# entn-at/tf-kaldi-speaker

Hardware: AMD Instinct MI355X
Metric: utterances/sec x-vector extraction (30-dim x 300-frame) (higher is better)
Workload: dtype f16+fp6-cross(f32-split); 1 GPU; tdnn x-vector (tdnn6_dense), statistics_pooling, 256 utt/GPU/step of 300 frames x 30 dims; batch_per_gpu=256, frames=300, node=tdnn6_dense, precision=f16f6, parallelism=utterance-shard x1, launch=stream launches

## Files before the change

### tf-kaldi-speaker_amd/csrc/api_forward.hip

```cpp
#include "xv_model.h"

using namespace xv;
using namespace xv::api;

namespace {

struct Run {
  xv_handle* h;
  const xv_plan* p;
  const float* feats;
  int feat_ld;
  float* out;
  char* ws;
  hipStream_t s;
  int f16;
  int B;
  const int32_t* off;
  char* raw(int64_t o) const { return o >= 0 ? ws + o : nullptr; }
  float* f32(int64_t o) const { return reinterpret_cast<float*>(raw(o)); }
  const float* in(int64_t o) const { return o == -2 ? feats : f32(o); }
  float* dst(const PlanStep& st) const { return st.out_off >= 0 ? f32(st.out_off) : out; }
  int* ovf() const { return static_cast<int*>(h->ovf_flag.p); }
};

// ... 45 lines not shown
    if (st.compact()) {
      a.arow = static_cast<const int32_t*>(r.p->d_rowmaps.p) + r.p->rowmap_off[st.arow];
      a.a_pitch = L.cin;
      a.a_off = L.mode == 1 ? 0 : (Sin + 1) * L.cin;
    }
    a.ntaps = L.mode == 1 ? 3 : 1;
    a.ktap = L.mode == 1 ? 3 * L.cin : (L.mode == 2 ? L.cin : L.Fin * L.cin);
    a.tap_stride = Sin * L.cin;
    a.cin = a.K;
  }
  if (op.in1 > 0) { a.R = r.in(st.in1_off); a.ldr = L.cout; }
  if (st.fuse_att == 1) {
    a.Y = nullptr;
    a.att_part = r.f32(st.out_off);
    a.att_ld = st.att_ld;
    a.att_heads = d.att_num_heads;
    a.att_q = static_cast<const float*>(h->query_eff.p);
  } else if (st.fuse_att == 2) {
    a.Y = nullptr;
    a.pool_part = r.f32(st.out_off);
    a.pool_row2utt = static_cast<const int32_t*>(r.p->d_row2utt.p);
    a.pool_slotbase = static_cast<const int32_t*>(r.p->d_slotbase.p);
    a.pool_w = r.f32(st.att_w_off);
    a.pool_heads = d.att_num_heads;
    a.pool_split = d.att_split_value;
    a.pool_dvh = d.att_split_value ? L.cout / d.att_num_heads : L.cout;
    a.pool_odim = h->pool_dim / 2;
  }
  if (st.fuse_pool) {
    a.Y = nullptr;
    a.pool_part = r.f32(st.out_off);
    a.pool_row2utt = static_cast<const int32_t*>(r.p->d_row2utt.p);
    a.pool_slotbase = static_cast<const int32_t*>(r.p->d_slotbase.p);
  }
  if (st.out_sb_off >= 0) {
    a.Ysb = r.raw(st.out_sb_off);
    a.ldsb = sb_ld(L.cout);
    if (st.out_off < 0 && !st.to_out) a.Y = nullptr;
  }
  return a;
}

int gemm_clear_border(const Run& r, const PlanStep& st, const Layer& L, const Value& vo) {
  xv_handle* h = r.h;
  const size_t head = (size_t)vo.grid_S + 1;
  const size_t rows0 = st.grid_cover && L.mode != 4 ? head : (st.grid_cover ? 0 : (size_t)st.rows_out + vo.grid_S);
  if (st.compact() || st.trows()) {
    XV_HIP(h, launch_grid_zero_border(r.p->dev_offsets(st.lvl_out), r.B, st.frames_out, vo.grid_F, vo.grid_S, L.cout / 4,
                                      sb_ld(L.cout) / 4, r.f32(st.out_off), r.raw(st.out_sb_off), r.s));
  } else if (rows0 > 0) {
    if (st.out_off >= 0) XV_HIP(h, hipMemsetAsync(r.raw(st.out_off), 0, rows0 * L.cout * 4, r.s));
    if (st.out_sb_off >= 0) XV_HIP(h, hipMemsetAsync(r.raw(st.out_sb_off), 0, rows0 * sb_ld(L.cout) * 4, r.s));
  }
  return XV_OK;
}

int launch_conv0(const Run& r, const PlanStep& st, const Layer& L, const Value& vo, GemmArgs& a) {
  xv_handle* h = r.h;
  if (st.scratch_off < 0) return fail(h, XV_ERR_STATE, "conv0 has no scratch");
  a.cin = 32; a.K = 32;
  const bool direct = L.use_split && !st.to_out && st.stage == L.final_stage() && L.cout % 8 == 0 &&
                      (st.out_sb_off < 0 || L.cout % 32 == 0) && L.cout <= 256 && L.wdir.p;
  if (direct) {
    XV_HIP(h, launch_conv0_direct(r.feats, r.feat_ld, r.off, r.B, L.Fout, vo.grid_S, L.cout, st.M, static_cast<const float*>(L.wdir.p),
                                  L.act, L.d_alpha(), r.f32(st.out_off), r.raw(st.out_sb_off), sb_ld(L.cout), r.f16, r.ovf(),
                                  a.sb_mul, r.s));
  } else if (L.use_split) {
    XV_HIP(h, launch_im2col2d_sb(r.feats, r.feat_ld, r.off, r.B, L.Fout, vo.grid_S, st.M, r.raw(st.scratch_off), r.f16, r.ovf(), r.s));
    a.Xsb = r.raw(st.scratch_off); a.ldsbx = 32; a.Wsb = L.wsb.p; a.Wfr = L.wfr.p;
    XV_HIP(h, launch_gemm_bf16x3(a, r.s));
  } else {
    XV_HIP(h, launch_im2col2d_f32(r.feats, r.feat_ld, r.off, r.B, L.Fout, vo.grid_S, st.M, r.f32(st.scratch_off), r.s));
    a.X = r.f32(st.scratch_off); a.ldx = 32;
    XV_HIP(h, launch_gemm_f32(a, true, r.s));
  }
  return XV_OK;
}

int launch_first_layer(const Run& r, const PlanStep& st, const Layer& L, GemmArgs& a) {
  xv_handle* h = r.h;
  if (st.scratch_off < 0) return fail(h, XV_ERR_STATE, "im2col layer has no scratch");
  a.Xsb = r.raw(st.scratch_off);
  a.Wsb = L.wsb.p; a.Wfr = L.wfr.p;
  if (L.cin_pad) {
    XV_HIP(h, launch_im2col_sb(r.feats, r.feat_ld, L.cin, 1, st.rows_in, r.raw(st.scratch_off), L.cin_pad, r.f16, r.ovf(), r.s));
    a.ldsbx = L.cin_pad;
    a.cin = L.cin_pad;
    a.K = L.w * L.cin_pad;
    a.ysb_f6 = st.out_f6 ? 1 : 0;
  } else {
    XV_HIP(h, launch_im2col_sb(r.feats, r.feat_ld, L.cin, L.w, st.M, r.raw(st.scratch_off), L.Kpad, r.f16, r.ovf(), r.s));
    a.ldsbx = L.Kpad;
    a.cin = a.K;
  }
  if (r.f16) XV_HIP(h, launch_feat_utt_guard(r.feats, r.feat_ld, L.cin, r.off, r.B, r.ovf(), r.s));
  XV_HIP(h, launch_gemm_bf16x3(a, r.s));
  return XV_OK;
}

int launch_two_unit(const Run& r, const PlanStep& st, const Op& op, const Layer& L, GemmArgs& a) {
  xv_handle* h = r.h;
  if (st.in0_sb_off < 0 || st.scratch_off < 0) return fail(h, XV_ERR_STATE, "f16f6 layer %s has no input / scratch", L.kernel_name.c_str());
  if (st.in_f6) {
    a.Xsb = r.raw(st.in0_sb_off);
  } else {
    XV_HIP(h, launch_f6_from_sb(r.raw(st.in0_sb_off), r.raw(st.scratch_off), st.rows_in, sb_ld(L.cin) / 32, r.s));
    a.Xsb = r.raw(st.scratch_off);
    XV_HIP(h, hipMemsetAsync(r.raw(st.scratch_off) + st.rows_in * (int64_t)sb_ld(L.cin) * 4, 0, (size_t)8 * sb_ld(L.cin) * 4, r.s));
  }
  a.ysb_f6 = st.out_f6 ? 1 : 0;
  a.ldsbx = sb_ld(L.cin);
  a.Wfr = L.wf6m.p;
  a.Wx6 = L.wf6x.p;
  if (st.trows()) {
    const int64_t Sin = h->values[op.in0].grid_S;
    a.a_pitch = 0; a.a_off = 0; a.arow = nullptr; a.ntaps = 0; a.ktap = 0; a.tap_stride = 0;
    a.ldsbx = Sin * L.cin;
    a.cin = 3 * L.cin;
    a.K = 9 * L.cin;
    a.nbin = L.Fout;
    a.bin_x_bytes = (int64_t)L.cin * 4;
    if (a.Ysb) a.Ysb = static_cast<char*>(a.Ysb) + (int64_t)a.ldsb * 4;
    if (a.Y) a.Y += a.ldy;
    if (a.R) a.R += a.ldr;
  }
  if (st.tail_mt > 0 && st.scratch2_off >= 0) {
    a.tail_mt = st.tail_mt;
    a.ksplit = st.ksplit;
    a.partial = r.f32(st.scratch2_off);
  }
  XV_HIP(h, launch_gemm_f16f6(a, r.s));
  return XV_OK;
}

int launch_split(const Run& r, const PlanStep& st, const Layer& L, GemmArgs& a) {
  xv_handle* h = r.h;
  if (st.in0_sb_off < 0) return fail(h, XV_ERR_STATE, "split layer %s has no split-blocked input", L.kernel_name.c_str());
  a.Xsb = r.raw(st.in0_sb_off);
  a.ldsbx = L.mode == 0 ? sb_ld(L.cin) : 0;
  a.Wsb = L.wsb.p; a.Wfr = L.wfr.p;
  a.ysb_f6 = st.out_f6 ? 1 : 0;
  if (st.tail_mt > 0 && st.scratch_off >= 0) {
    a.tail_mt = st.tail_mt;
    a.ksplit = st.ksplit;
    a.partial = r.f32(st.scratch_off);
  }
  XV_HIP(h, launch_gemm_bf16x3(a, r.s));
  return XV_OK;
}

int launch_fp32(const Run& r, const PlanStep& st, const Op& op, const Layer& L, GemmArgs& a) {
  xv_handle* h = r.h;
  if (st.ksplit > 1 && st.scratch_off >= 0) {
    a.ksplit = st.ksplit;
    a.partial = r.f32(st.scratch_off);
  }
  const bool aligned = op.in0 != 0 && (a.ldx % 4 == 0) && (a.K % 4 == 0);
  if (L.mode != 0 && !aligned)
    return fail(h, XV_ERR_UNSUPPORTED, "resnet convolution %s needs channel counts that are multiples of 4", L.kernel_name.c_str());
  XV_HIP(h, launch_gemm_f32(a, aligned, r.s));
  return XV_OK;
}

int run_gemm(const Run& r, const PlanStep& st, const Op& op) {
  xv_handle* h = r.h;
  const Layer& L = h->layers[op.layer];
  const Value& vo = h->values[op.out];
  GemmArgs a = gemm_args(r, st, op, L);
  int rc = vo.grid_F > 0 ? gemm_clear_border(r, st, L, vo) : XV_OK;
  if (rc != XV_OK) return rc;
  if (L.mode == 4) rc = launch_conv0(r, st, L, vo, a);
  else if (L.im2col) rc = launch_first_layer(r, st, L, a);
  else if (L.use_f6) rc = launch_two_unit(r, st, op, L, a);
  else if (L.use_split) rc = launch_split(r, st, L, a);
  else rc = launch_fp32(r, st, op, L, a);
  if (rc != XV_OK) return rc;
  if (st.unpad_to_out)
    XV_HIP(h, launch_grid_unpad_n(r.f32(st.out_off), r.p->dev_offsets(st.lvl_out), r.B, vo.grid_F, vo.grid_S, vo.cols, st.frames_out,
// ... 208 lines not shown
```

### tf-kaldi-speaker_amd/csrc/api_weights.hip

```cpp
#include "xv_model.h"

using namespace xv;
using namespace xv::api;

namespace {

constexpr double kBnEps = 1e-3;

uint16_t f32_to_bf16_rn(float f) {
  uint32_t u;
  memcpy(&u, &f, 4);
  if ((u & 0x7fffffffu) > 0x7f800000u) return (uint16_t)((u >> 16) | 0x40);
  u += 0x7fffu + ((u >> 16) & 1u);
  return (uint16_t)(u >> 16);
}
float bf16_to_f32(uint16_t b) {
  uint32_t u = (uint32_t)b << 16;
  float f;
  memcpy(&f, &u, 4);
  return f;
}
uint16_t f32_to_f16_rn(float f) {
  const _Float16 h = (_Float16)f;
  uint16_t u;
// ... 244 lines not shown
  return XV_OK;
}

void choose_kernels(xv_handle* h) {
  for (const Op& op : h->ops) {
    if (op.kind != OP_GEMM) continue;
    Layer& L = h->layers[op.layer];
    const Value& vin = h->values[op.in0];
    const bool bf = h->desc.precision != XV_PREC_F32;
    if (L.mode == 0) {
      L.im2col = bf && op.in0 == 0;
      L.cin_pad = (L.im2col && L.w <= 9) ? (int)align_up(L.cin, 32) : 0;
      L.use_split = L.im2col || (bf && vin.frame_level && (L.w == 1 || (L.cin % 32 == 0 && L.w <= 9)));
      L.use_f6 = h->desc.precision == XV_PREC_F16F6 && L.use_split && !L.im2col && (L.w == 5 || L.w == 7 || L.w == 9) &&
                 L.cin % 128 == 0 && L.cout % 4 == 0;
    } else {
      L.use_split = bf && (L.mode == 4 || L.cin % 32 == 0);
      L.use_f6 = h->desc.precision == XV_PREC_F16F6 && h->opt_grid_f6 && L.mode == 1 && L.use_split && L.sw == 1 && L.st == 1 &&
                 L.cin % 128 == 0 && L.cout % 128 == 0;
    }
    if (L.use_f6 && f6_block_spread(h, op, L) > kF6MaxSpread) L.use_f6 = false;
  }
  if (h->desc.precision == XV_PREC_F16X3 || h->desc.precision == XV_PREC_F16F6) {
    for (const Op& op : h->ops) {
      if (op.kind == OP_GEMM) {
        Layer& L = h->layers[op.layer];
        L.in_exp = (L.use_split && !L.im2col && L.mode != 4 && op.in0 > 0) ? h->values[op.in0].sb_exp : 0;
        L.out_exp = act_exponent(h, L);
        h->values[op.out].sb_exp = L.out_exp;
      } else if (op.kind == OP_GRID_MAXPOOL) {
        h->values[op.out].sb_exp = h->values[op.in0].sb_exp;
      }
    }
  }
}

}

extern "C" {

int xv_finalize(xv_handle* h) {
  if (!h) return fail(nullptr, XV_ERR_INVALID, "xv_finalize: null handle");
  std::lock_guard<std::mutex> lk(h->mu);
  if (h->finalized) return XV_OK;
  for (const auto& kv : h->tensors)
    if (!kv.second.set) return fail(h, XV_ERR_MISSING_TENSOR, "variable '%s' was never set", kv.first.c_str());
  choose_kernels(h);
  DeviceGuard g(h->device);
  if (!g.ok) return fail(h, XV_ERR_HIP, "cannot select HIP device %d", h->device);
  for (auto& L : h->layers) {
    const int rc = upload_layer(h, L);
    if (rc != XV_OK) return rc;
  }
  if (h->desc.pooling_type == XV_POOL_SELF_ATTENTION) {
    const auto& q = T(h, std::string(h->desc.network_type == XV_NET_ETDNN ? "etdnn/" : "tdnn/") + "attention/query").data;
    XV_HIP(h, h->query.alloc(q.size() * sizeof(float)));
    XV_HIP(h, hipMemcpy(h->query.p, q.data(), q.size() * sizeof(float), hipMemcpyHostToDevice));
    {
      const int H = h->desc.att_num_heads, dkh = h->att_dk_h;
      h->key_npad = (int)align_up(h->att_dk, 128);
      std::vector<float> qe((size_t)H * h->key_npad, 0.f);
      for (int hd = 0; hd < H; ++hd)
        for (int d = 0; d < dkh; ++d) {
          const int n = h->desc.att_split_key ? hd * dkh + d : d;
          qe[(size_t)hd * h->key_npad + n] = q[(size_t)hd * dkh + d];
        }
      XV_HIP(h, h->query_eff.alloc(qe.size() * sizeof(float)));
      XV_HIP(h, hipMemcpy(h->query_eff.p, qe.data(), qe.size() * sizeof(float), hipMemcpyHostToDevice));
    }
    if (h->desc.att_apply_nonlinear) {
      const int n = h->pool_dim;
      std::vector<double> s, t;
      bn_fold(h, h->post_bn_scope, n, s, t);
      std::vector<float> vec((size_t)3 * n, 0.f);
      for (int i = 0; i < n; ++i) { vec[i] = (float)s[i]; vec[(size_t)n + i] = (float)t[i]; }
      if (!h->post_alpha_name.empty()) {
        const auto& a = T(h, h->post_alpha_name).data;
        for (int i = 0; i < n; ++i) vec[(size_t)2 * n + i] = a[i];
      }
      XV_HIP(h, h->post_vec.alloc(vec.size() * sizeof(float)));
      XV_HIP(h, hipMemcpy(h->post_vec.p, vec.data(), vec.size() * sizeof(float), hipMemcpyHostToDevice));
    }
  }
  XV_HIP(h, h->ovf_flag.alloc((kFlagWords + kFeatMaxSlots) * sizeof(int)));
  XV_HIP(h, hipMemset(h->ovf_flag.p, 0, (kFlagWords + kFeatMaxSlots) * sizeof(int)));
  XV_HIP(h, hipDeviceSynchronize());
  for (auto& kv : h->tensors) { kv.second.data.clear(); kv.second.data.shrink_to_fit(); }
  h->finalized = true;
  return XV_OK;
}

int xv_check_overflow(xv_handle* h, int reset) {
  if (!h) return fail(nullptr, XV_ERR_INVALID, "xv_check_overflow: null handle");
  if (!h->finalized || !h->ovf_flag.p) return 0;
  DeviceGuard g(h->device);
  std::vector<int32_t> w((size_t)kFlagWords + kFeatMaxSlots);
  XV_HIP(h, hipMemcpy(w.data(), h->ovf_flag.p, w.size() * sizeof(int32_t), hipMemcpyDeviceToHost));
  int32_t v[2] = {w[0], w[1]};
  for (int i = 0; i < kFeatMaxSlots; ++i) v[1] = std::max(v[1], w[(size_t)kFlagWords + i]);
  if (w[kUttSmallWord]) v[1] = w[kUttSmallWord];
  if (reset) XV_HIP(h, hipMemset(h->ovf_flag.p, 0, w.size() * sizeof(int32_t)));
  return xv_flags_decode(v);
}

int xv_flags_decode(const int32_t* flags) {
  if (!flags) return XV_ERR_INVALID;
  if (flags[0]) return 1;
  if (flags[1] > 0) {
    float mx;
    memcpy(&mx, &flags[1], 4);
    if (mx < 0.00390625f) return 2;
  }
  return 0;
}

int xv_flags_async(xv_handle* h, int32_t* host_flags, void* stream) {
  if (!h || !host_flags) return fail(h, XV_ERR_INVALID, "xv_flags_async: null argument");
  if (!h->finalized || !h->ovf_flag.p) { host_flags[0] = host_flags[1] = 0; return XV_OK; }
  DeviceGuard g(h->device);
  hipStream_t s = static_cast<hipStream_t>(stream);
  hipPointerAttribute_t attr;
  if (hipPointerGetAttributes(&attr, host_flags) == hipSuccess && attr.type == hipMemoryTypeHost) {
    XV_HIP(h, launch_flags_snapshot(static_cast<int*>(h->ovf_flag.p), host_flags, s));
    return XV_OK;
  }
  (void)hipGetLastError();
  XV_HIP(h, launch_flags_snapshot(static_cast<int*>(h->ovf_flag.p), static_cast<int*>(h->ovf_flag.p) + 2, s));
  XV_HIP(h, hipMemcpyAsync(host_flags, static_cast<int*>(h->ovf_flag.p) + 2, 2 * sizeof(int32_t), hipMemcpyDeviceToHost, s));
  return XV_OK;
}

}
```

### tf-kaldi-speaker_amd/csrc/gemm_f32.hip

```cpp
#include <mutex>

#include "xv_epilogue.h"

namespace xv {

constexpr int BM = 128, BN = 128, BK = 32;
constexpr int LDT = BK + 4;
constexpr int TILE_F = BM * LDT;

template <int FORM>
__global__ __launch_bounds__(256, 2) void gemm_f32_kernel(GemmArgs p, int nMt, int nNt, int kper) {
  extern __shared__ __attribute__((aligned(16))) float smem[];
  float* As = smem;
  float* Bs = smem + 2 * TILE_F;

  const int tid = threadIdx.x;
  const int lane = tid & 63, wave = tid >> 6;
  const int wm = wave >> 1, wn = wave & 1;
  const int r32 = lane & 31, h = lane >> 5;

  const int ntiles = nMt * nNt;
  const int slice = blockIdx.x / ntiles;
  const int tile = xcd_remap(blockIdx.x - slice * ntiles, ntiles);
  const int mt = tile / nNt, nt = tile - mt * nNt;
// ... 32 lines not shown
        }
      } else {
        const int m = m0 + row;
        f32x4 v = {0.f, 0.f, 0.f, 0.f};
        if (m < p.M) {
#pragma unroll
          for (int e = 0; e < 4; ++e) {
            const int kk = k + e;
            if (kk < p.K) {
              const int dr = kk / p.cin;
              v[e] = p.X[(int64_t)(m + dr) * p.ldx + (kk - dr * p.cin)];
            }
          }
        }
        ra[i] = v;
      }
    }
  };
  auto store_tiles = [&](int buf) {
#pragma unroll
    for (int i = 0; i < 4; ++i) {
      const int row = lr + 32 * i;
      *reinterpret_cast<f32x4*>(As + buf * TILE_F + row * LDT + c4 * 4) = ra[i];
      *reinterpret_cast<f32x4*>(Bs + buf * TILE_F + row * LDT + c4 * 4) = rb[i];
    }
  };

  f32x16 acc[2][2];
#pragma unroll
  for (int i = 0; i < 2; ++i)
#pragma unroll
    for (int j = 0; j < 2; ++j)
#pragma unroll
      for (int e = 0; e < 16; ++e) acc[i][j][e] = 0.f;

  load_tiles(kt0);
  store_tiles(0);
  __syncthreads();

  const float* a_base = As + (wm * 64 + r32) * LDT + 4 * h;
  const float* b_base = Bs + (wn * 64 + r32) * LDT + 4 * h;

  for (int kt = kt0; kt < nk; ++kt) {
    const int cur = (kt - kt0) & 1;
    if (kt + 1 < nk) load_tiles(kt + 1);
    const float* ap = a_base + cur * TILE_F;
    const float* bp = b_base + cur * TILE_F;
#pragma unroll
    for (int q = 0; q < BK / 8; ++q) {
      f32x4 a0 = *reinterpret_cast<const f32x4*>(ap + q * 8);
      f32x4 a1 = *reinterpret_cast<const f32x4*>(ap + 32 * LDT + q * 8);
      f32x4 b0 = *reinterpret_cast<const f32x4*>(bp + q * 8);
      f32x4 b1 = *reinterpret_cast<const f32x4*>(bp + 32 * LDT + q * 8);
#pragma unroll
      for (int j = 0; j < 4; ++j) {
        acc[0][0] = __builtin_amdgcn_mfma_f32_32x32x2f32(b0[j], a0[j], acc[0][0], 0, 0, 0);
        acc[0][1] = __builtin_amdgcn_mfma_f32_32x32x2f32(b0[j], a1[j], acc[0][1], 0, 0, 0);
        acc[1][0] = __builtin_amdgcn_mfma_f32_32x32x2f32(b1[j], a0[j], acc[1][0], 0, 0, 0);
        acc[1][1] = __builtin_amdgcn_mfma_f32_32x32x2f32(b1[j], a1[j], acc[1][1], 0, 0, 0);
      }
    }
    if (kt + 1 < nk) store_tiles(cur ^ 1);
    __syncthreads();
  }

  store_wave_tile(p, acc, m0 + wm * 64, n0 + wn * 64, lane, wave, reinterpret_cast<char*>(smem));
}

__global__ void splitk_reduce_kernel(GemmArgs p) {
  const int64_t total = (int64_t)p.M * p.N;
  for (int64_t i = (int64_t)blockIdx.x * blockDim.x + threadIdx.x; i < total; i += (int64_t)gridDim.x * blockDim.x) {
    const int m = (int)(i / p.N), n = (int)(i - (int64_t)m * p.N);
    float acc = 0.f;
    for (int s = 0; s < p.ksplit; ++s) acc += p.partial[((int64_t)s * p.M + m) * p.Npad + n];
    bool zero;
    const int orow = out_row(p, m, zero);
    if (orow < 0) continue;
    float v = fmaf(acc, p.scale[n], p.shift[n]);
    if (p.R) v += p.R[(int64_t)orow * p.ldr + n];
    p.Y[(int64_t)orow * p.ldy + n] = zero ? 0.f : apply_act(v, p.act, p.alpha ? p.alpha[n] : 0.f);
  }
}

int gemm_f32_ksplit(int M, int Kpad, int Npad) {
  if (M > 512) return 1;
  const int tiles = ((M + BM - 1) / BM) * (Npad / BN), nk = Kpad / BK;
  int s = 512 / (tiles > 0 ? tiles : 1);
  if (s > nk / 4) s = nk / 4;
  return s < 2 ? 1 : s;
}

hipError_t launch_gemm_f32(const GemmArgs& a, bool aligned, hipStream_t s) {
  if (a.M <= 0) return hipSuccess;
  const int nMt = (a.M + BM - 1) / BM, nNt = a.Npad / BN;
  const int ks = (a.ksplit > 1 && a.partial && !a.Ysb && !a.pool_part) ? a.ksplit : 1;
  const int nk_all = a.Kpad / BK;
  const int kper = (nk_all + ks - 1) / ks;
  const size_t smem = (size_t)4 * TILE_F * sizeof(float);
  static std::mutex init_mu;
  static bool attr_set[64] = {};
  int dev = 0;
  if (hipGetDevice(&dev) != hipSuccess) dev = 0;
  std::lock_guard<std::mutex> init_lock(init_mu);
  if (!attr_set[dev & 63]) {
    hipError_t e = hipFuncSetAttribute(reinterpret_cast<const void*>(gemm_f32_kernel<2>),
                                       hipFuncAttributeMaxDynamicSharedMemorySize, (int)smem);
    if (e != hipSuccess) return e;
    e = hipFuncSetAttribute(reinterpret_cast<const void*>(gemm_f32_kernel<1>),
                                       hipFuncAttributeMaxDynamicSharedMemorySize, (int)smem);
    if (e != hipSuccess) return e;
    e = hipFuncSetAttribute(reinterpret_cast<const void*>(gemm_f32_kernel<0>),
                            hipFuncAttributeMaxDynamicSharedMemorySize, (int)smem);
    if (e != hipSuccess) return e;
    attr_set[dev & 63] = true;
  }
  GemmArgs b = a;
  b.ksplit = ks;
  dim3 grid(nMt * nNt * ks), block(256);
  if (aligned && a.a_pitch)
    hipLaunchKernelGGL(gemm_f32_kernel<2>, grid, block, smem, s, b, nMt, nNt, kper);
  else if (aligned)
    hipLaunchKernelGGL(gemm_f32_kernel<1>, grid, block, smem, s, b, nMt, nNt, kper);
  else
    hipLaunchKernelGGL(gemm_f32_kernel<0>, grid, block, smem, s, b, nMt, nNt, kper);
  hipError_t e = hipGetLastError();
  if (e != hipSuccess || ks == 1) return e;
  const int64_t total = (int64_t)a.M * a.N;
  const int blocks = (int)((total + 255) / 256 > 1024 ? 1024 : (total + 255) / 256);
  hipLaunchKernelGGL(splitk_reduce_kernel, dim3(blocks), dim3(256), 0, s, b);
  return hipGetLastError();
}

}
```

### tf-kaldi-speaker_amd/csrc/pool.hip

```cpp
#include "xv_epilogue.h"

namespace xv {


__device__ __forceinline__ float act_apply(float v, int act, float alpha) {
  switch (act) {
    case ACT_RELU: return fmaxf(v, 0.0f);
    case ACT_LRELU: return fmaxf(v, kLreluAlpha * v);
    case ACT_PRELU: return fmaxf(v, 0.0f) + alpha * (v - fabsf(v)) * 0.5f;
    case ACT_TANH: return tanhf(v);
    default: return v;
  }
}

__device__ __forceinline__ float wave_sum(float v) {
#pragma unroll
  for (int o = 32; o > 0; o >>= 1) v += __shfl_xor(v, o, 64);
  return v;
}
__device__ __forceinline__ float wave_max(float v) {
#pragma unroll
  for (int o = 32; o > 0; o >>= 1) v = fmaxf(v, __shfl_xor(v, o, 64));
  return v;
}
// ... 307 lines not shown
  const int h = min(split ? oc / dvh : oc / (odim / H), H - 1);
  const int r0 = off0[b] - b * ctx, r1 = off0[b + 1] - (b + 1) * ctx;
  const int t0 = r0 >> 6, t1 = (r1 - 1) >> 6;
  const int64_t base = (int64_t)slotbase[b];
  float mean = 0.f;
  for (int t = t0; t <= t1; ++t) mean += part[((base + t) * 2) * odim + oc];
  float var = 0.f;
  for (int t = t0; t <= t1; ++t) {
    const float w = s0[(base + t) * H + h];
    const float d = w > 0.f ? part[((base + t) * 2) * odim + oc] / w - mean : 0.f;
    var += part[((base + t) * 2 + 1) * odim + oc] + w * d * d;
  }
  var = var <= kVarFloor ? kVarFloor : var;
  out[(int64_t)b * ldo + oc] = mean;
  out[(int64_t)b * ldo + odim + oc] = sqrtf(var);
}

hipError_t launch_att_pool_finalize(const float* part, const float* s0, int odim, int H, int dvh, int split,
                                    const int32_t* off0, int B, int ctx, const int32_t* slotbase, float* out, int64_t ldo,
                                    hipStream_t s) {
  if (B <= 0) return hipSuccess;
  hipLaunchKernelGGL(att_pool_finalize_kernel, dim3((odim + 255) / 256, B), dim3(256), 0, s, part, s0, odim, H, dvh, split,
                     off0, ctx, slotbase, out, ldo);
  return hipGetLastError();
}

__global__ void att_weights_out_kernel(const float* __restrict__ scores, int H,
                                       const int32_t* __restrict__ off0, int ctx, float* __restrict__ out) {
  const int h = blockIdx.x, b = blockIdx.y;
  const int r0 = off0[b] - b * ctx, r1 = off0[b + 1] - (b + 1) * ctx;
  const int L = r1 - r0;
  for (int t = threadIdx.x; t < L; t += blockDim.x)
    out[((int64_t)b * H + h) * L + t] = scores[(int64_t)(r0 + t) * H + h];
}

hipError_t launch_att_weights_out(const float* scores, int H, const int32_t* off0, int B, int ctx,
                                  float* out, hipStream_t s) {
  if (B <= 0) return hipSuccess;
  hipLaunchKernelGGL(att_weights_out_kernel, dim3(H, B), dim3(256), 0, s, scores, H, off0, ctx, out);
  return hipGetLastError();
}

__global__ void im2col_sb_kernel(const float* __restrict__ x, int64_t ldx, int cin, int K, int64_t rows,
                                 char* __restrict__ out, int ldsb, int f16, int* __restrict__ ovf) {
  const int pairs = ldsb >> 1;
  const int64_t total = rows * pairs;
  float mx = 0.f;
  for (int64_t i = (int64_t)blockIdx.x * blockDim.x + threadIdx.x; i < total; i += (int64_t)gridDim.x * blockDim.x) {
    const int64_t m = i / pairs;
    const int k = (int)(i - m * pairs) * 2;
    float v[2];
#pragma unroll
    for (int e = 0; e < 2; ++e) {
      const int kk = k + e;
      const int dr = kk / cin;
      v[e] = kk < K ? x[(m + dr) * ldx + (kk - dr * cin)] : 0.f;
    }
    uint32_t hi, lo;
    split2(v[0], v[1], hi, lo, f16);
    if (f16) ovf_report(ovf, fmaxf(fabsf(v[0]), fabsf(v[1])));
    mx = fmaxf(mx, fmaxf(fabsf(v[0]), fabsf(v[1])));
    char* blk = out + m * (int64_t)ldsb * 4 + (k >> 5) * 128 + (k & 31) * 2;
    *reinterpret_cast<uint32_t*>(blk) = hi;
    *reinterpret_cast<uint32_t*>(blk + 64) = lo;
  }
  if (f16 && ovf) {
#pragma unroll
    for (int o = 32; o > 0; o >>= 1) mx = fmaxf(mx, __shfl_xor(mx, o, 64));
    if ((threadIdx.x & 63) == 0)
      reinterpret_cast<float*>(ovf + kFlagWords)[blockIdx.x * 4 + (threadIdx.x >> 6)] = (mx <= 3.0e38f) ? mx : 0.f;
  }
}

hipError_t launch_im2col_sb(const float* x, int64_t ldx, int cin, int w, int64_t rows, void* out_sb, int ldsb, int f16,
                            int* ovf, hipStream_t s) {
  if (rows <= 0) return hipSuccess;
  const int64_t total = rows * (ldsb >> 1);
  const int blocks = (int)((total + 255) / 256 > kFeatMaxSlots / 4 ? kFeatMaxSlots / 4 : (total + 255) / 256);
  hipLaunchKernelGGL(im2col_sb_kernel, dim3(blocks), dim3(256), 0, s, x, ldx, cin, w * cin, rows,
                     static_cast<char*>(out_sb), ldsb, f16, ovf);
  return hipGetLastError();
}

__global__ void affine_act_kernel(const float* __restrict__ x, int64_t ldx, int64_t rows, int C,
                                  const float* __restrict__ scale, const float* __restrict__ shift,
                                  const float* __restrict__ alpha, int act, float* __restrict__ y,
                                  int64_t ldy) {
  const int64_t n = rows * C;
  for (int64_t i = (int64_t)blockIdx.x * blockDim.x + threadIdx.x; i < n; i += (int64_t)gridDim.x * blockDim.x) {
    const int64_t r = i / C;
    const int c = (int)(i - r * C);
    const float v = fmaf(x[r * ldx + c], scale ? scale[c] : 1.f, shift ? shift[c] : 0.f);
    y[r * ldy + c] = act_apply(v, act, alpha ? alpha[c] : 0.f);
  }
}

hipError_t launch_affine_act(const float* x, int64_t ldx, int64_t rows, int C, const float* scale,
                             const float* shift, const float* alpha, int act, float* y, int64_t ldy,
                             hipStream_t s) {
  const int64_t n = rows * C;
  if (n <= 0) return hipSuccess;
  const int blocks = (int)((n + 255) / 256 > 2048 ? 2048 : (n + 255) / 256);
  hipLaunchKernelGGL(affine_act_kernel, dim3(blocks), dim3(256), 0, s, x, ldx, rows, C, scale, shift, alpha,
                     act, y, ldy);
  return hipGetLastError();
}

__global__ __launch_bounds__(256) void l2_scale_kernel(const float* __restrict__ x, int64_t rows, int C,
                                                       float factor, float* __restrict__ y) {
  const int lane = threadIdx.x & 63;
  const int64_t r = (int64_t)blockIdx.x * 4 + (threadIdx.x >> 6);
  if (r >= rows) return;
  float s = 0.f;
  for (int c = lane; c < C; c += 64) {
    const float v = x[r * C + c];
    s = fmaf(v, v, s);
  }
  s = wave_sum(s);
  const float inv = rsqrtf(fmaxf(s, 1e-12f)) * factor;
  for (int c = lane; c < C; c += 64) y[r * C + c] = x[r * C + c] * inv;
}

hipError_t launch_l2_scale(const float* x, int64_t rows, int C, float factor, float* y, hipStream_t s) {
  if (rows <= 0) return hipSuccess;
  hipLaunchKernelGGL(l2_scale_kernel, dim3((unsigned)((rows + 3) / 4)), dim3(256), 0, s, x, rows, C, factor, y);
  return hipGetLastError();
}

__global__ void flags_snapshot_kernel(int* __restrict__ dev, int* __restrict__ host) {
  float* part = reinterpret_cast<float*>(dev + kFlagWords);
  __shared__ float wmax[16];
  float mx = 0.f;
  for (int i = threadIdx.x; i < kFeatMaxSlots; i += 1024) {
    mx = fmaxf(mx, part[i]);
    part[i] = 0.f;
  }
#pragma unroll
  for (int o = 32; o > 0; o >>= 1) mx = fmaxf(mx, __shfl_xor(mx, o, 64));
  if ((threadIdx.x & 63) == 0) wmax[threadIdx.x >> 6] = mx;
  __syncthreads();
  if (threadIdx.x == 0) {
    for (int i = 1; i < 16; ++i) mx = fmaxf(mx, wmax[i]);
    host[0] = dev[0];
    host[1] = dev[kUttSmallWord] ? dev[kUttSmallWord] : __float_as_int(fmaxf(mx, __int_as_float(dev[1])));
    dev[0] = 0;
    dev[1] = 0;
    dev[kUttSmallWord] = 0;
    __threadfence_system();
  }
}

__global__ void feat_utt_guard_kernel(const float* __restrict__ x, int64_t ldx, int cin, const int32_t* __restrict__ offs,
                                      int* __restrict__ flags) {
  __shared__ float wmax[16];
  const int64_t r0 = offs[blockIdx.x];
  const int n = (int)(offs[blockIdx.x + 1] - r0) * cin;
  float mx = 0.f;
  if (ldx == cin) {
    const float* p = x + r0 * ldx;
    for (int i = threadIdx.x; i < n; i += blockDim.x) mx = fmaxf(mx, fabsf(p[i]));
  } else {
    for (int i = threadIdx.x; i < n; i += blockDim.x) {
      const int r = i / cin;
      mx = fmaxf(mx, fabsf(x[(r0 + r) * ldx + (i - r * cin)]));
    }
  }
// ... 43 lines not shown
```

### tf-kaldi-speaker_amd/csrc/xv_kernels.h

```cpp
#pragma once
#include <hip/hip_runtime.h>
#include <stdint.h>

#include <string>

#include "../../include/xvec_hip.h"

namespace xv {

enum Act : int { ACT_NONE = 0, ACT_RELU = 1, ACT_LRELU = 2, ACT_PRELU = 3, ACT_TANH = 4 };

constexpr float kLreluAlpha = 0.2f;
constexpr int kFlagWords = 8, kUttSmallWord = 4, kFeatMaxSlots = 32768;
constexpr float kVarFloor = 1e-12f;

struct GemmArgs {
  const float* X;
  int64_t ldx;
  int cin;
  int M;
  int K;
  int N;
  const float* Wt;
  int Kpad;
  int Npad;
  const float* scale;
  const float* shift;
  const float* alpha;
  int act;
  const int32_t* rowmap;
  float* Y;
  int64_t ldy;
  const void* Xsb;
  int64_t ldsbx;
  void* Ysb;
  int ldsb;
  const void* Wsb;
  const void* Wfr = nullptr;
  const void* Wx6 = nullptr;
  int ysb_f6 = 0;
  int slab3 = 1;
  int* ovf = nullptr;
  int nbin = 0;
  int64_t bin_x_bytes = 0;
  float sb_mul = 1.f;
  int f16 = 0;
  long long* trace = nullptr;
  int ksplit;
  int raw;
  float* partial;
  int tail_mt = 0;
  float* pool_part;
  const int32_t* pool_row2utt;
  const int32_t* pool_slotbase;
  int64_t a_pitch;
  int64_t a_off;
  int64_t tap_stride;
  int ntaps;
  int ktap;
  const int32_t* arow;
  const float* R;
  int64_t ldr;
  const float* att_q = nullptr;
  float* att_part = nullptr;
  int64_t att_ld = 0;
  int att_heads = 0;
  const float* pool_w = nullptr;
  int pool_heads = 0;
  int pool_split = 0;
  int pool_dvh = 0;
  int pool_odim = 0;
};

hipError_t launch_gemm_f32(const GemmArgs& a, bool aligned, hipStream_t s);

int gemm_f32_ksplit(int M, int Kpad, int Npad);

int64_t gemm_bf16x3_tail_plan(int M, int Kpad, int Npad, int w, int* tail_mt, int* splits, int cb_quant = 1);

hipError_t launch_im2col_sb(const float* x, int64_t ldx, int cin, int w, int64_t rows, void* out_sb, int ldsb, int f16,
                            int* ovf, hipStream_t s);

hipError_t launch_gemm_bf16x3(const GemmArgs& a, hipStream_t s);
hipError_t launch_gemm_f16f6(const GemmArgs& a, hipStream_t s);
hipError_t launch_f6v2_tail_reduce(const GemmArgs& a, int nMain, hipStream_t s);
hipError_t launch_f6_from_sb(const void* sb, void* out, int64_t rows, int nblk, hipStream_t s);

hipError_t launch_build_rowmap(const int32_t* off0, int B, int ctx_in, int w, int32_t* rowmap, int M,
                               hipStream_t s);

hipError_t launch_stat_pool(const float* x, int64_t ldx, int C, const int32_t* off0, int B, int ctx,
                            float* out, int64_t ldo, hipStream_t s);

hipError_t launch_build_row2utt(const int32_t* off0, int B, int ctx, int32_t* row2utt, int M, hipStream_t s);
hipError_t launch_pool_finalize(const float* part, int C, const int32_t* off0, int B, int ctx,
                                const int32_t* slotbase, float* out, int64_t ldo, hipStream_t s);

hipError_t launch_build_rowmap_grid(const int32_t* off0, int B, int rows_per_t, int Fout, int So, int cover, int32_t* rowmap,
                                    int64_t M, hipStream_t s);
hipError_t launch_build_rowmap_grid_ts(const int32_t* off_in, const int32_t* off_out, int B, int rows_per_t, int Fout, int So,
                                       int ktime, int32_t* rowmap, int64_t M, hipStream_t s);
hipError_t launch_build_rowmap_grid_compact(const int32_t* off_in, const int32_t* off_out, int B, int Sin, int So, int Fout,
                                            int sw, int st, int ktime, int32_t* arow, int32_t* rowmap, int64_t M, int64_t Mpad,
                                            hipStream_t s);
hipError_t launch_grid_zero_border(const int32_t* off0, int B, int64_t frames, int F, int S, int chunks_y, int chunks_sb,
                                   float* y, void* ysb, hipStream_t s);
hipError_t launch_build_rowmap_rows(const int32_t* off0, int B, int32_t* rowmap, int64_t M, hipStream_t s);
hipError_t launch_build_rowmap_trows(const int32_t* off0, int B, int So, int32_t* rowmap, int64_t M, hipStream_t s);
hipError_t launch_build_rowmap_interior(const int32_t* off0, int B, int F, int S, int32_t* rowmap, int64_t M, hipStream_t s);
hipError_t launch_im2col2d_sb(const float* x, int64_t ldx, const int32_t* off0, int B, int F, int S, int64_t P, void* out_sb,
                              int f16, int* ovf, hipStream_t s);
hipError_t launch_im2col2d_f32(const float* x, int64_t ldx, const int32_t* off0, int B, int F, int S, int64_t P, float* out,
                               hipStream_t s);
hipError_t launch_conv0_direct(const float* x, int64_t ldx, const int32_t* off0, int B, int F, int S, int C, int64_t P,
                               const float* wdir, int act, const float* alpha, float* y, void* ysb, int ldsb, int f16, int* ovf,
                               float sb_mul, hipStream_t s);
hipError_t launch_grid_maxpool3x3(const float* x, const int32_t* off0, int B, int F, int S, int C, int64_t P, float* y,
                                  void* ysb, int ldsb, int f16, int* ovf, float sb_mul, hipStream_t s);
hipError_t launch_grid_unpad_n(const float* grid, const int32_t* off0, int B, int F, int S, int C, int64_t frames, float* out,
                               hipStream_t s);

hipError_t launch_cmn_select(const float* x, int64_t ld, int dim, const int32_t* off, int B, double* prefix,
                             const int32_t* src, int64_t out_rows, int window, int center, int min_window, float* out,
                             hipStream_t s);

int mfcc_create(const xv_mfcc_opts* opts, int device, xv_mfcc** out, std::string* err);
void mfcc_destroy(xv_mfcc* m);
int mfcc_num_frames(const xv_mfcc* m, int64_t num_samples, int64_t* out);
int mfcc_device(const xv_mfcc* m);
int mfcc_num_ceps(const xv_mfcc* m);
hipError_t launch_mfcc(xv_mfcc* m, const int16_t* wave, const int64_t* sample_off, const int32_t* frame_off, int B, float* out,
                       int64_t ld, hipStream_t s);
hipError_t launch_vad_energy(const float* feats, int64_t ld, const int32_t* frame_off, int B, float threshold, float mean_scale,
                             int context, float proportion, float* vad, hipStream_t s);
int fbank_create(const xv_fbank_opts* opts, int device, xv_fbank** out, std::string* err);
void fbank_destroy(xv_fbank* m);
int fbank_num_frames(const xv_fbank* m, int64_t num_samples, int64_t* out);
int fbank_device(const xv_fbank* m);
int fbank_num_feats(const xv_fbank* m);
hipError_t launch_fbank(xv_fbank* m, const int16_t* wave, const int64_t* sample_off, const int32_t* frame_off, int B, float* out,
                        int64_t ld, float* log_energy, hipStream_t s);

hipError_t launch_length_norm(const float* x, int64_t ldx, int64_t rows, int dim, int scaleup, float* y, int64_t ldy,
                              hipStream_t s);
hipError_t launch_speaker_mean(const float* x, int64_t ldx, int dim, const int32_t* spk_off, const int32_t* utt,
                               int64_t num_spk, float* out, int64_t ldo, hipStream_t s);

hipError_t launch_score_prepare_rows(const float* x, int64_t ldx, int64_t rows, int dim, const float* mean, int normalize,
                                     float eps, float* y, int64_t ldy, hipStream_t s);
hipError_t launch_score_matrix(const float* a, int64_t lda, int n, const float* b, int64_t ldb, int m, int d,
                               const float* a_sub, int b_offset, float* out, int64_t ldo, hipStream_t s);
hipError_t launch_score_histogram(const float* a, int64_t lda, int n, const int32_t* la, const float* b, int64_t ldb, int m,
                                  const int32_t* lb, int d, int self, int nbins, unsigned long long* hs,
                                  unsigned long long* hd, hipStream_t s);
hipError_t launch_score_pairs(const float* a, int64_t lda, int n, const float* b, int64_t ldb, int m, int d, const int32_t* ia,
                              const int32_t* ib, int64_t npairs, float* out, hipStream_t s);

hipError_t launch_plda_rows(const float* u, int64_t ldu, int64_t rows, int d, int norm, int side, int pack_second,
                            const double* tables, const double* logdet, const int32_t* table_index, int num_tables,
                            float* rows_out, int64_t ldr, float* packed, int64_t ldp, float* bias, hipStream_t s);
hipError_t launch_plda_matrix(const float* a, int64_t lda, int n, const float* row_bias, const float* b, int64_t ldb, int m,
                              const float* col_bias, int k, float* out, int64_t ldo, hipStream_t s);
hipError_t launch_plda_histogram(const float* a, int64_t lda, int n, const float* row_bias, const int32_t* la, const float* b,
                                 int64_t ldb, int m, const float* col_bias, const int32_t* lb, int k, double lo, double hi,
                                 int nbins, unsigned long long* hs, unsigned long long* hd, hipStream_t s);
// ... 87 lines not shown
```

Measured before the change: 221,900 utterances/s.

## Fuse feature staging with per-utterance guard and add small-M f32 GEMM

Adds a per-utterance feature staging kernel for the first layer. It splits features into the hi/lo storage format and computes the per-utterance max/overflow flags in the same pass, replacing the separate im2col launch and guard launch. Long utterances need an extra fold kernel and a larger flag buffer. It also adds a K-parallel MFMA f32 GEMM path for small M (at most 512) that reduces across waves in shared memory, aimed at the small post-pooling dense layers that underfill the 128x128 tiled kernel.

```diff
diff --git a/tf-kaldi-speaker_amd/csrc/api_forward.hip b/tf-kaldi-speaker_amd/csrc/api_forward.hip
--- a/tf-kaldi-speaker_amd/csrc/api_forward.hip
+++ b/tf-kaldi-speaker_amd/csrc/api_forward.hip
@@ -151,8 +151,17 @@
   if (st.scratch_off < 0) return fail(h, XV_ERR_STATE, "im2col layer has no scratch");
   a.Xsb = r.raw(st.scratch_off);
   a.Wsb = L.wsb.p; a.Wfr = L.wfr.p;
+  bool guarded = false;
   if (L.cin_pad) {
-    XV_HIP(h, launch_im2col_sb(r.feats, r.feat_ld, L.cin, 1, st.rows_in, r.raw(st.scratch_off), L.cin_pad, r.f16, r.ovf(), r.s));
+    const std::vector<int32_t>& ho = r.p->lvl_offsets[0];
+    guarded = feat_stage_sb_ok(L.cin_pad, r.B) && (int)ho.size() == r.B + 1 && ho[r.B] == st.rows_in;
+    if (guarded) {
+      int max_len = 0;
+      for (int b = 0; b < r.B; ++b) max_len = std::max(max_len, ho[b + 1] - ho[b]);
+      XV_HIP(h, launch_feat_stage_sb(r.feats, r.feat_ld, L.cin, r.off, r.B, max_len, r.raw(st.scratch_off), L.cin_pad, r.f16, r.ovf(), r.s));
+    } else {
+      XV_HIP(h, launch_im2col_sb(r.feats, r.feat_ld, L.cin, 1, st.rows_in, r.raw(st.scratch_off), L.cin_pad, r.f16, r.ovf(), r.s));
+    }
     a.ldsbx = L.cin_pad;
     a.cin = L.cin_pad;
     a.K = L.w * L.cin_pad;
@@ -162,7 +171,7 @@
     a.ldsbx = L.Kpad;
     a.cin = a.K;
   }
-  if (r.f16) XV_HIP(h, launch_feat_utt_guard(r.feats, r.feat_ld, L.cin, r.off, r.B, r.ovf(), r.s));
+  if (r.f16 && !guarded) XV_HIP(h, launch_feat_utt_guard(r.feats, r.feat_ld, L.cin, r.off, r.B, r.ovf(), r.s));
   XV_HIP(h, launch_gemm_bf16x3(a, r.s));
   return XV_OK;
 }
diff --git a/tf-kaldi-speaker_amd/csrc/api_weights.hip b/tf-kaldi-speaker_amd/csrc/api_weights.hip
--- a/tf-kaldi-speaker_amd/csrc/api_weights.hip
+++ b/tf-kaldi-speaker_amd/csrc/api_weights.hip
@@ -350,8 +350,8 @@
       XV_HIP(h, hipMemcpy(h->post_vec.p, vec.data(), vec.size() * sizeof(float), hipMemcpyHostToDevice));
     }
   }
-  XV_HIP(h, h->ovf_flag.alloc((kFlagWords + kFeatMaxSlots) * sizeof(int)));
-  XV_HIP(h, hipMemset(h->ovf_flag.p, 0, (kFlagWords + kFeatMaxSlots) * sizeof(int)));
+  XV_HIP(h, h->ovf_flag.alloc(kFlagBufWords * sizeof(int)));
+  XV_HIP(h, hipMemset(h->ovf_flag.p, 0, kFlagBufWords * sizeof(int)));
   XV_HIP(h, hipDeviceSynchronize());
   for (auto& kv : h->tensors) { kv.second.data.clear(); kv.second.data.shrink_to_fit(); }
   h->finalized = true;
diff --git a/tf-kaldi-speaker_amd/csrc/gemm_f32.hip b/tf-kaldi-speaker_amd/csrc/gemm_f32.hip
--- a/tf-kaldi-speaker_amd/csrc/gemm_f32.hip
+++ b/tf-kaldi-speaker_amd/csrc/gemm_f32.hip
@@ -138,6 +138,95 @@
   }
 }
 
+constexpr int SG_TM = 32, SG_TN = 16, SG_WAVES = 8, SG_KS = 32, SG_PF = 4;
+
+__global__ __launch_bounds__(SG_WAVES * 64) void gemm_f32_seg_kernel(GemmArgs p, int nNt, int vec_out) {
+  __shared__ __attribute__((aligned(16))) float red[SG_WAVES][SG_TM * SG_TN];
+  const int tid = threadIdx.x;
+  const int lane = tid & 63, wave = tid >> 6;
+  const int i16 = lane & 15, g = lane >> 4;
+  const int mt = blockIdx.x / nNt, nt = blockIdx.x - mt * nNt;
+  const int m0 = mt * SG_TM, n0 = nt * SG_TN;
+  const int nks = p.Kpad / SG_KS;
+
+  const float* wrow = p.Wt + (int64_t)(n0 + i16) * p.Kpad + 8 * g;
+  const float* xrow0 = p.X + (int64_t)min(m0 + i16, p.M - 1) * p.ldx;
+  const float* xrow1 = p.X + (int64_t)min(m0 + 16 + i16, p.M - 1) * p.ldx;
+  const f32x4 z = {0.f, 0.f, 0.f, 0.f};
+  f32x4 rw[SG_PF][2], rx0[SG_PF][2], rx1[SG_PF][2];
+  auto load_step = [&](int s, int i) {
+    const int k = min(s, nks - 1) * SG_KS;
+#pragma unroll
+    for (int c = 0; c < 2; ++c) {
+      const int kx = min(k + 8 * g + 4 * c, p.K - 4);
+      rw[i][c] = *reinterpret_cast<const f32x4*>(wrow + k + 4 * c);
+      rx0[i][c] = *reinterpret_cast<const f32x4*>(xrow0 + kx);
+      rx1[i][c] = *reinterpret_cast<const f32x4*>(xrow1 + kx);
+    }
+  };
+  auto keep_here = [] {
+    asm volatile("" ::: "memory");
+    __builtin_amdgcn_sched_barrier(0);
+  };
+
+  f32x4 acc0 = z, acc1 = z;
+#pragma unroll
+  for (int i = 0; i < SG_PF; ++i) load_step(wave + i * SG_WAVES, i);
+  keep_here();
+  for (int s = wave; s < nks; s += SG_PF * SG_WAVES) {
+#pragma unroll
+    for (int i = 0; i < SG_PF; ++i) {
+      const int si = s + i * SG_WAVES;
+      const bool in = si < nks;
+      f32x4 w[2], x0[2], x1[2];
+#pragma unroll
+      for (int c = 0; c < 2; ++c) {
+        const bool inx = in && si * SG_KS + 8 * g + 4 * c < p.K;
+        w[c] = in ? rw[i][c] : z;
+        x0[c] = inx ? rx0[i][c] : z;
+        x1[c] = inx ? rx1[i][c] : z;
+      }
+      load_step(si + SG_PF * SG_WAVES, i);
+      keep_here();
+#pragma unroll
+      for (int c = 0; c < 2; ++c)
+#pragma unroll
+        for (int j = 0; j < 4; ++j) {
+          acc0 = __builtin_amdgcn_mfma_f32_16x16x4f32(w[c][j], x0[c][j], acc0, 0, 0, 0);
+          acc1 = __builtin_amdgcn_mfma_f32_16x16x4f32(w[c][j], x1[c][j], acc1, 0, 0, 0);
+        }
+    }
+  }
+
+  *reinterpret_cast<f32x4*>(&red[wave][i16 * SG_TN + 4 * g]) = acc0;
+  *reinterpret_cast<f32x4*>(&red[wave][(16 + i16) * SG_TN + 4 * g]) = acc1;
+  __syncthreads();
+  if (tid >= SG_TM * SG_TN / 4) return;
+  const int ml = tid >> 2, q = tid & 3;
+  f32x4 acc = *reinterpret_cast<const f32x4*>(&red[0][ml * SG_TN + 4 * q]);
+#pragma unroll
+  for (int w = 1; w < SG_WAVES; ++w) acc += *reinterpret_cast<const f32x4*>(&red[w][ml * SG_TN + 4 * q]);
+  const int m = m0 + ml, n = n0 + 4 * q;
+  if (m >= p.M || n >= p.N) return;
+  float* y = p.Y + (int64_t)m * p.ldy + n;
+  if (vec_out) {
+    const f32x4 sc = *reinterpret_cast<const f32x4*>(p.scale + n), sh = *reinterpret_cast<const f32x4*>(p.shift + n);
+    const f32x4 al = p.alpha ? *reinterpret_cast<const f32x4*>(p.alpha + n) : z;
+    f32x4 v;
+#pragma unroll
+    for (int e = 0; e < 4; ++e) v[e] = apply_act(fmaf(acc[e], sc[e], sh[e]), p.act, al[e]);
+    *reinterpret_cast<f32x4*>(y) = v;
+  } else {
+#pragma unroll
+    for (int e = 0; e < 4; ++e)
+      if (n + e < p.N) y[e] = apply_act(fmaf(acc[e], p.scale[n + e], p.shift[n + e]), p.act, p.alpha ? p.alpha[n + e] : 0.f);
+  }
+}
+
+static bool seg_form(const GemmArgs& a, bool aligned) {
+  return aligned && !a.a_pitch && a.M <= 512 && a.Y && !a.rowmap && !a.R && !a.Ysb && !a.pool_part && !a.att_part && !a.raw;
+}
+
 int gemm_f32_ksplit(int M, int Kpad, int Npad) {
   if (M > 512) return 1;
   const int tiles = ((M + BM - 1) / BM) * (Npad / BN), nk = Kpad / BK;
@@ -148,6 +237,14 @@
 
 hipError_t launch_gemm_f32(const GemmArgs& a, bool aligned, hipStream_t s) {
   if (a.M <= 0) return hipSuccess;
+  if (seg_form(a, aligned)) {
+    const int nMt = (a.M + SG_TM - 1) / SG_TM, nNt = (a.N + SG_TN - 1) / SG_TN;
+    const int vec_out = (a.N & 3) == 0 && (a.ldy & 3) == 0 && (reinterpret_cast<uintptr_t>(a.Y) & 15) == 0 &&
+                        (reinterpret_cast<uintptr_t>(a.scale) & 15) == 0 && (reinterpret_cast<uintptr_t>(a.shift) & 15) == 0 &&
+                        (reinterpret_cast<uintptr_t>(a.alpha) & 15) == 0;
+    hipLaunchKernelGGL(gemm_f32_seg_kernel, dim3(nMt * nNt), dim3(SG_WAVES * 64), 0, s, a, nNt, vec_out);
+    return hipGetLastError();
+  }
   const int nMt = (a.M + BM - 1) / BM, nNt = a.Npad / BN;
   const int ks = (a.ksplit > 1 && a.partial && !a.Ysb && !a.pool_part) ? a.ksplit : 1;
   const int nk_all = a.Kpad / BK;
diff --git a/tf-kaldi-speaker_amd/csrc/pool.hip b/tf-kaldi-speaker_amd/csrc/pool.hip
--- a/tf-kaldi-speaker_amd/csrc/pool.hip
+++ b/tf-kaldi-speaker_amd/csrc/pool.hip
@@ -413,6 +413,117 @@
   return hipGetLastError();
 }
 
+constexpr int kStageRows = 128, kStageSingleRows = 512;
+
+template <bool VEC2>
+__global__ __launch_bounds__(1024) void feat_stage_sb_kernel(const float* __restrict__ x, int64_t ldx, int cin,
+                                                             const int32_t* __restrict__ offs, char* __restrict__ out,
+                                                             int ldsb, int f16, int* __restrict__ flags, int single) {
+  __shared__ float wmax[16];
+  const int b = blockIdx.y;
+  const int64_t r0 = offs[b];
+  const int len = (int)(offs[b + 1] - r0);
+  const int row_begin = single ? 0 : blockIdx.x * kStageRows;
+  if (row_begin >= len) return;
+  const int row_end = single ? len : min(len, row_begin + kStageRows);
+  const int lpr = ldsb >> 3, rpp = blockDim.x / lpr;
+  const int rs = threadIdx.x / lpr, c8 = threadIdx.x - rs * lpr;
+  const int k0 = 8 * c8;
+  float mx = 0.f;
+  bool bad = false;
+  if (rs < rpp) {
+    const float* src = x + (r0 + row_begin + rs) * ldx + k0;
+    char* dst = out + (r0 + row_begin + rs) * (int64_t)ldsb * 4 + (c8 >> 2) * 128 + (c8 & 3) * 16;
+    for (int row = row_begin + rs; row < row_end; row += rpp, src += (int64_t)rpp * ldx, dst += (int64_t)rpp * ldsb * 4) {
+      float v[8];
+#pragma unroll
+      for (int e = 0; e < 8; e += 2) {
+        if (VEC2 && k0 + e + 1 < cin) {
+          const float2 t = *reinterpret_cast<const float2*>(src + e);
+          v[e] = t.x;
+          v[e + 1] = t.y;
+        } else {
+          v[e] = k0 + e < cin ? src[e] : 0.f;
+          v[e + 1] = k0 + e + 1 < cin ? src[e + 1] : 0.f;
+        }
+      }
+      uint32_t hi[4], lo[4];
+#pragma unroll
+      for (int e = 0; e < 4; ++e) {
+        split2(v[2 * e], v[2 * e + 1], hi[e], lo[e], f16);
+        const float m2 = fmaxf(fabsf(v[2 * e]), fabsf(v[2 * e + 1]));
+        bad |= !(m2 <= kF16Max);
+        mx = fmaxf(mx, m2);
+      }
+      *reinterpret_cast<uint4*>(dst) = make_uint4(hi[0], hi[1], hi[2], hi[3]);
+      *reinterpret_cast<uint4*>(dst + 64) = make_uint4(lo[0], lo[1], lo[2], lo[3]);
+    }
+  }
+  if (!f16 || !flags) return;
+  if (bad) flags[0] = 1;
+#pragma unroll
+  for (int o = 32; o > 0; o >>= 1) mx = fmaxf(mx, __shfl_xor(mx, o, 64));
+  if ((threadIdx.x & 63) == 0) wmax[threadIdx.x >> 6] = mx;
+  __syncthreads();
+  if (threadIdx.x == 0) {
+    for (int i = 1; i < (int)(blockDim.x >> 6); ++i) mx = fmaxf(mx, wmax[i]);
+    if (single) {
+      reinterpret_cast<float*>(flags + kFlagWords)[b] = (mx <= 3.0e38f) ? mx : 0.f;
+      if (mx > 0.f && mx < 0.00390625f) flags[kUttSmallWord] = __float_as_int(mx);
+    } else if (mx > 0.f) {
+      atomicMax(flags + kFlagWords + kFeatMaxSlots + b, __float_as_int(mx));
+    }
+  }
+}
+
+__global__ __launch_bounds__(1024) void feat_utt_fold_kernel(int* __restrict__ flags, int batch) {
+  __shared__ float wmax[16], wsmall[16];
+  int* utt = flags + kFlagWords + kFeatMaxSlots;
+  float mx = 0.f, small = 0.f;
+  for (int i = threadIdx.x; i < batch; i += 1024) {
+    const float v = __int_as_float(utt[i]);
+    utt[i] = 0;
+    if (v > 0.f && v < 0.00390625f) small = fmaxf(small, v);
+    mx = fmaxf(mx, v <= 3.0e38f ? v : 0.f);
+  }
+#pragma unroll
+  for (int o = 32; o > 0; o >>= 1) {
+    mx = fmaxf(mx, __shfl_xor(mx, o, 64));
+    small = fmaxf(small, __shfl_xor(small, o, 64));
+  }
+  if ((threadIdx.x & 63) == 0) {
+    wmax[threadIdx.x >> 6] = mx;
+    wsmall[threadIdx.x >> 6] = small;
+  }
+  __syncthreads();
+  if (threadIdx.x == 0) {
+    for (int i = 1; i < 16; ++i) {
+      mx = fmaxf(mx, wmax[i]);
+      small = fmaxf(small, wsmall[i]);
+    }
+    if (small > 0.f) flags[kUttSmallWord] = __float_as_int(small);
+    if (mx > 0.f) atomicMax(flags + 1, __float_as_int(mx));
+  }
+}
+
+bool feat_stage_sb_ok(int ldsb, int batch) { return ldsb % 32 == 0 && ldsb <= 2048 && batch <= kUttMaxSlots && batch <= kFeatMaxSlots; }
+
+hipError_t launch_feat_stage_sb(const float* x, int64_t ldx, int cin, const int32_t* offsets_dev, int batch, int max_len,
+                                void* out_sb, int ldsb, int f16, int* flags, hipStream_t s) {
+  if (batch <= 0 || max_len <= 0) return hipSuccess;
+  if (!feat_stage_sb_ok(ldsb, batch)) return hipErrorInvalidValue;
+  const int single = max_len <= kStageSingleRows;
+  const dim3 grid(single ? 1 : (max_len + kStageRows - 1) / kStageRows, batch), block(single ? 1024 : 256);
+  if (ldx % 2 == 0 && (reinterpret_cast<uintptr_t>(x) & 7) == 0)
+    hipLaunchKernelGGL(feat_stage_sb_kernel<true>, grid, block, 0, s, x, ldx, cin, offsets_dev, static_cast<char*>(out_sb), ldsb, f16, flags, single);
+  else
+    hipLaunchKernelGGL(feat_stage_sb_kernel<false>, grid, block, 0, s, x, ldx, cin, offsets_dev, static_cast<char*>(out_sb), ldsb, f16, flags, single);
+  const hipError_t e = hipGetLastError();
+  if (e != hipSuccess || !f16 || !flags || single) return e;
+  hipLaunchKernelGGL(feat_utt_fold_kernel, dim3(1), dim3(1024), 0, s, flags, batch);
+  return hipGetLastError();
+}
+
 __global__ void affine_act_kernel(const float* __restrict__ x, int64_t ldx, int64_t rows, int C,
                                   const float* __restrict__ scale, const float* __restrict__ shift,
                                   const float* __restrict__ alpha, int act, float* __restrict__ y,
diff --git a/tf-kaldi-speaker_amd/csrc/xv_kernels.h b/tf-kaldi-speaker_amd/csrc/xv_kernels.h
--- a/tf-kaldi-speaker_amd/csrc/xv_kernels.h
+++ b/tf-kaldi-speaker_amd/csrc/xv_kernels.h
@@ -12,6 +12,8 @@
 
 constexpr float kLreluAlpha = 0.2f;
 constexpr int kFlagWords = 8, kUttSmallWord = 4, kFeatMaxSlots = 32768;
+constexpr int kUttMaxSlots = 32768;
+constexpr int kFlagBufWords = kFlagWords + kFeatMaxSlots + kUttMaxSlots;
 constexpr float kVarFloor = 1e-12f;
 
 struct GemmArgs {
@@ -81,6 +83,10 @@
 hipError_t launch_im2col_sb(const float* x, int64_t ldx, int cin, int w, int64_t rows, void* out_sb, int ldsb, int f16,
                             int* ovf, hipStream_t s);
 
+bool feat_stage_sb_ok(int ldsb, int batch);
+hipError_t launch_feat_stage_sb(const float* x, int64_t ldx, int cin, const int32_t* offsets_dev, int batch, int max_len,
+                                void* out_sb, int ldsb, int f16, int* flags, hipStream_t s);
+
 hipError_t launch_gemm_bf16x3(const GemmArgs& a, hipStream_t s);
 hipError_t launch_gemm_f16f6(const GemmArgs& a, hipStream_t s);
 hipError_t launch_f6v2_tail_reduce(const GemmArgs& a, int nMain, hipStream_t s);
```

Measured after the change: 225,400 utterances/s, median of 6. +1.6%, better.
